# scychon/openmm_drudeNose

Measured on AMD Instinct MI355X. Metric: integrator steps/sec at 1M Drude pairs, higher is better.
Workload: dtype f64; 1 GPU; SWM4-NDP water box, 1000000 molecules = 5000000 particle slots, 1000000 Drude pairs, 1 temperature group (+ molecular-COM and Drude thermostats), TGNH mode, mixed precision, numNHChains=1, hard wall 0.02 nm, harness force call-out inside the timed region (harness_force: lattice); harness_force=lattice, precision=mixed, variant=resident, hipgraph=False, parallelism=particle-sharded x1 (whole molecules), one KE all-reduce per step, slots_per_gpu=5000000

## Files before the change

openmm_drudenose_amd/csrc/tgnh_kernels.hip:

```cpp
#include "tgnh_tile_device.h"

#ifdef TGNH_TRACE
TGNH_TRACE_READERS(tgnh_debug_read_trace, tgnh_debug_clear_trace)
extern "C" int tgnh_debug_read_chain_trace(unsigned long long* out) {
    return (int)hipMemcpyFromSymbol(out, HIP_SYMBOL(tgnh::g_chain_trace), sizeof(unsigned long long) * 8);
}
#endif

namespace tgnh {


size_t tile_lds_bytes(int precision, int ops, bool hardwall, bool use_com) {
    (void)use_com;
    const size_t m4 = (precision == TGNH_PREC_SINGLE) ? 16 : 32;
    const bool hw = hardwall && (ops & (OP_DRIFT | OP_MOVE));
    size_t b = (size_t)(TBLOCK / 64) * (MAX_GROUPS + 2) * 8;
    if ((ops & (OP_SCALE | OP_KE)) || hw) b = m4 * (TILE_SLOTS + TILE_RES);
    if (hw) b += m4 * TILE_SLOTS;
    return b;
}

#ifndef TGNH_MINWAVES
#define TGNH_MINWAVES 1
#endif
// ... 626 lines not shown
            const double dx = ix[pl] - v.x, dy = iy[pl] - v.y, dz = iz[pl] - v.z;
            const double mass1 = mass, mass2 = im[pl];
            const double mu = mass1 * mass2 * rcp_(mass1 + mass2);
            const double d = (dx * dx + dy * dy + dz * dz) * mu;
            ke_drude += d;
            val -= d;
        }
#pragma unroll
        for (int b = 0; b < GB; b++) ke_g[b] += (g == (uint32_t)b) ? val : 0.0;
        __builtin_amdgcn_fence(__ATOMIC_RELEASE, "wavefront");
        __builtin_amdgcn_wave_barrier();
        __builtin_amdgcn_fence(__ATOMIC_ACQUIRE, "wavefront");
    };

    int w = __builtin_amdgcn_readfirstlane((int)blockIdx.x * (TBLOCK / 64) + wv);
    Bounds b0{}, b1{}, b2{};
    WaveIn<PREC> A, B;
    PatternWord pw;
    auto load = [&](const Bounds& b, WaveIn<PREC>& in) {
        const bool patterned = pw.of(a, (uint32_t)b.y >> 8, lane);
        wave_load<PREC, OPS>(a, b.ws, b.n, patterned, pw.word, lane, in);
    };
    if (w < nw) { bounds(w, b0); load(b0, A); }
    if (w + stride < nw) bounds(w + stride, b1);
    while (w < nw) {
        if (w + 2 * stride < nw) bounds(w + 2 * stride, b2);
        if (w + stride < nw) load(b1, B);
        work(A, b0);
        w += stride;
        if (w >= nw) break;
        if (w + 2 * stride < nw) bounds(w + 2 * stride, b0);
        if (w + stride < nw) load(b2, A);
        work(B, b1);
        w += stride;
        b1 = b0; b0 = b2;
    }
#pragma unroll
    for (int b = 0; b < GB; b++) ke_g[b] = wave_sum(ke_g[b]);
    ke_com = wave_sum(ke_com);
    ke_drude = wave_sum(ke_drude);
    if (lane == 0) {
#pragma unroll
        for (int b = 0; b < GB; b++) sred[wv][b] = ke_g[b];
        sred[wv][GB] = ke_com;
        sred[wv][GB + 1] = ke_drude;
    }
    __syncthreads();
    if (tid < GB + 2) {
        double t = 0.0;
#pragma unroll
        for (int k = 0; k < TBLOCK / 64; k++) t += sred[k][tid];
        const int b = tid < GB ? tid : G + (tid - GB);
        if (tid >= GB || tid < G) {
            if (a.tail_sum) {
                unsigned long long* cell = a.rows + row_word((int)blockIdx.x, 2 * b);
                const unsigned long long bits = (unsigned long long)__double_as_longlong(t), tg = (unsigned long long)(gen0 + 1u) << 32;
                __hip_atomic_store(cell, tg | (bits & 0xffffffffull), __ATOMIC_RELAXED, __HIP_MEMORY_SCOPE_SYSTEM);
                __hip_atomic_store(cell + 64, tg | (bits >> 32), __ATOMIC_RELAXED, __HIP_MEMORY_SCOPE_SYSTEM);
            } else a.partials[(size_t)blockIdx.x * (G + 2) + b] = t;
        }
    }
    if (a.tail_sum && blockIdx.x == 0) {
        __shared__ double s_tail[TBLOCK / 64][GB + 2];
        const int NT = G + 2;
        double acc[GB + 2];
#pragma unroll
        for (int b = 0; b < GB + 2; b++) acc[b] = 0.0;
        const bool ok = collect_rows<GB, false, TBLOCK>(a, tid, (int)gridDim.x, NT, (unsigned long long)(gen0 + 1u), acc);
        if (!ok) atomicOr(a.status, 16u);
#pragma unroll
        for (int b = 0; b < GB + 2; b++) {
            if (b < NT) {
                const double t = wave_sum(acc[b]);
                if (lane == 0) s_tail[wv][b] = t;
            }
        }
        const bool all_ok = __syncthreads_and(ok ? 1 : 0) != 0;
        if (tid < NT) {
            double t = 0.0;
#pragma unroll
            for (int k = 0; k < TBLOCK / 64; k++) t += s_tail[k][tid];
            a.ke_red[tid] = all_ok ? t : __longlong_as_double(0x7ff8000000000000ll);
        }
        if (tid == 0) a.sync[1] = gen0 + 1u;
    }
}



enum : int { STEP_DEFER = 0, STEP_PLAIN_BEGIN = 1, STEP_PLAIN_END = 2, STEP_SPLIT_BEGIN = 3, STEP_SPLIT_END = 4, STEP_KINDS = 5 };
constexpr int step_ops1(int kind) {
    return (kind == STEP_DEFER || kind == STEP_PLAIN_END) ? (OP_KICK | OP_KE | OP_NOSTORE) : OP_KE;
}
constexpr int step_ops2(int kind) {
    return kind == STEP_DEFER ? (OP_PREKICK | OP_SCALE | OP_KICK | OP_DRIFT)
         : kind == STEP_PLAIN_BEGIN ? (OP_SCALE | OP_KICK | OP_DRIFT)
         : kind == STEP_PLAIN_END ? (OP_PREKICK | OP_SCALE)
         : kind == STEP_SPLIT_BEGIN ? (OP_SCALE | OP_KICK | OP_POSDELTA)
         : OP_SCALE;
}

template <int PREC, int GB, int KIND>
__global__ __launch_bounds__(TBLOCK, TGNH_MINWAVES) void step_kernel(const TileArgs a) {
    typedef typename Prec<PREC>::mixed mixed;
    constexpr int STEP_OPS1 = step_ops1(KIND), STEP_OPS2 = step_ops2(KIND);
    __shared__ double s_scale[MAX_GROUPS + 2];
    __shared__ double s_part[TBLOCK / 64][CHAIN_INLINE_SUM_NT];
    __shared__ double s_x[64 + XCHG_MAX_WORLD * CHAIN_INLINE_SUM_NT];
    __shared__ int s_go;
    __shared__ unsigned s_gen;
    __shared__ unsigned long long s_seq1;
    extern __shared__ __attribute__((aligned(16))) char smem[];
    const int tid = threadIdx.x, G = a.num_groups, NT = G + 2;
    const int grid = (int)gridDim.x;
    const bool chain_wave = tid < 64;
    const int itg = tid & 63;
    if (a.census) {
        if (tid == 0) {
            __hip_atomic_fetch_add(&a.sync[2], 1u, __ATOMIC_RELAXED, __HIP_MEMORY_SCOPE_AGENT);
            unsigned n = 0;
            while (__hip_atomic_load(&a.sync[2], __ATOMIC_RELAXED, __HIP_MEMORY_SCOPE_AGENT) < gridDim.x && ++n < CENSUS_SPIN_LIMIT)
                __builtin_amdgcn_s_sleep(16);
            if (__hip_atomic_load(&a.sync[2], __ATOMIC_RELAXED, __HIP_MEMORY_SCOPE_AGENT) < gridDim.x) atomicOr(&a.sync[3], 1u);
        }
        return;
    }
    TileEnv<PREC, GB> e;
    e.init(a, smem, s_scale, OpsOf<STEP_OPS2>::POS && a.hardwall != 0);
    auto tile_of = [&](int tt) { return a.reverse ? a.num_tiles - 1 - tt : tt; };

    unsigned gen0 = 0;
    unsigned long long seq0 = 0;
    Chain1Regs creg{};
    if (chain_wave) {
        gen0 = __hip_atomic_load(&a.sync[1], __ATOMIC_RELAXED, __HIP_MEMORY_SCOPE_AGENT);
        seq0 = __hip_atomic_load(a.chain.x.seq, __ATOMIC_RELAXED, __HIP_MEMORY_SCOPE_AGENT);
        if (itg < NT) creg = chain1_load(a.chain, a.st_in, itg);
    }

    TRACE(0);
    TileIn<PREC> cur;
    int tt = blockIdx.x;
    TilePattern tp;
    tile_load<PREC, STEP_OPS1>(a, tile_of(tt), cur, tp);
    for (;;) {
        tile_body<PREC, STEP_OPS1, GB>(a, e, cur, 4);
        if (tt + grid >= a.num_tiles) break;
        tt += grid;
        tile_load<PREC, STEP_OPS1>(a, tile_of(tt), cur, tp);
    }
    const int tt_last = tt;
    TRACE(1);
    MeetShared sh{s_scale, s_part, s_x, &s_go, &s_gen, &s_seq1, nullptr};
    if (!step_meet<PREC, GB>(a, e, gen0, seq0, creg, sh, [&] { tile_load<PREC, STEP_OPS2, STEP_OPS1>(a, tile_of(tt_last), cur, tp); }))
        return;
    e.s_com = (mixed)s_scale[G]; e.s_drude = (mixed)s_scale[G + 1];
    TRACE(9);

    tt = tt_last;
    for (bool held = true;; held = false) {
        tile_body<PREC, STEP_OPS2, GB>(a, e, cur, 0, held);
        if (tt - grid < 0) break;
        tt -= grid;
        tile_load<PREC, STEP_OPS2>(a, tile_of(tt), cur, tp);
    }
    TRACE(15);
}


template <int PREC, int GB, bool MULTI = false>
__global__ __launch_bounds__(WBLOCK) void wstep_kernel(const TileArgs a) {
    typedef typename Prec<PREC>::mixed mixed;
    static_assert(GB > 0, "register bins only");
    __shared__ double s_scale[MAX_GROUPS + 2];
    __shared__ double s_part[WBLOCK / 64][CHAIN_INLINE_SUM_NT];
    __shared__ double s_x[64 + XCHG_MAX_WORLD * CHAIN_INLINE_SUM_NT];
    __shared__ int s_go;
    __shared__ unsigned s_gen;
    __shared__ unsigned long long s_seq1;
    __shared__ mixed s_img[WBLOCK / 64][7][WAVE_SLOTS];
    __shared__ double s_block[256];
    const int tid = threadIdx.x, lane = tid & 63, G = a.num_groups, NT = G + 2;
    const int wv = __builtin_amdgcn_readfirstlane(tid >> 6);
    const bool chain_wave = tid < 64;
    const int itg = tid & 63;
    if (a.census) {
        if (tid == 0) {
            __hip_atomic_fetch_add(&a.sync[2], 1u, __ATOMIC_RELAXED, __HIP_MEMORY_SCOPE_AGENT);
            unsigned n = 0;
            while (__hip_atomic_load(&a.sync[2], __ATOMIC_RELAXED, __HIP_MEMORY_SCOPE_AGENT) < gridDim.x && ++n < CENSUS_SPIN_LIMIT)
                __builtin_amdgcn_s_sleep(16);
            if (__hip_atomic_load(&a.sync[2], __ATOMIC_RELAXED, __HIP_MEMORY_SCOPE_AGENT) < gridDim.x) atomicOr(&a.sync[3], 1u);
        }
        return;
    }
    TileEnv<PREC, GB> e;
    e.tid = tid; e.G = G; e.smem = nullptr; e.wbins0 = nullptr; e.s_scale = s_scale;
    e.clear_ke();
    WaveStep<PREC, GB> ws(a, &e, s_scale, &s_img[wv][0][0], lane);
    typedef WaveBounds Bounds;
    auto bounds = [&](const int ww, Bounds& b) { ws.bounds(ww, b); };
    auto load_vf = [&](const Bounds& b, WStepIn<PREC>& in) { ws.load_vf(b, in); };
    auto load_x = [&](const Bounds& b, WStepIn<PREC>& in) { ws.load_x(b, in); };
    auto prepare = [&](WStepIn<PREC>& t, const Bounds& bd, const bool ke) { ws.template prepare<true>(t, bd, ke); };
    auto finish = [&](WStepIn<PREC>& t, const Bounds& bd) { ws.finish(t, bd); };
    auto wfence = [] { WaveStep<PREC, GB>::wfence(); };

    unsigned gen0 = 0;
    unsigned long long seq0 = 0;
    Chain1Regs creg{};
    if (chain_wave) {
        gen0 = __hip_atomic_load(&a.sync[1], __ATOMIC_RELAXED, __HIP_MEMORY_SCOPE_AGENT);
        seq0 = __hip_atomic_load(a.chain.x.seq, __ATOMIC_RELAXED, __HIP_MEMORY_SCOPE_AGENT);
        if (itg < NT && !(MULTI && a.chain.L.C > 1)) creg = chain1_load(a.chain, a.st_in, itg);
    }
    if (MULTI && a.chain.L.C > 1 && tid < a.chain.L.total) s_block[tid] = a.st_in[tid];

    const int nw = a.num_wtiles, stride = (int)gridDim.x * (WBLOCK / 64);

    TRACE(0);
    const int w0 = __builtin_amdgcn_readfirstlane((int)blockIdx.x * (WBLOCK / 64) + wv);
    const bool have = w0 < nw;
    int w = w0;
    Bounds b0{}, b1{};
    WStepIn<PREC> cur;
    if (have) {
        bounds(w, b0);
        if (w + stride < nw) bounds(w + stride, b1);
        load_vf(b0, cur);
    }
    while (have) {
#ifdef TGNH_TRACE
        if (w == w0) { asm volatile("s_waitcnt vmcnt(0)" ::: "memory"); TRACE(3); }
#endif
        prepare(cur, b0, true);
#ifdef TGNH_TRACE
        if (w == w0) TRACE(4);
#endif
        if (w + stride >= nw) break;
        wfence();
        w += stride;
        b0 = b1;
        if (w + stride < nw) bounds(w + stride, b1);
        load_vf(b0, cur);
    }
    const int w_last = w;
    TRACE(1);
    MeetShared sh{s_scale, s_part, s_x, &s_go, &s_gen, &s_seq1, s_block};
    if (!step_meet<PREC, GB, true, WBLOCK, MULTI>(a, e, gen0, seq0, creg, sh, [&] {
            if (have) {
                load_x(b0, cur);
                if (w_last - stride >= 0) bounds(w_last - stride, b1);
            }
        })) return;

    TRACE(9);
    if (have) {
        w = w_last;
        finish(cur, b0);
        TRACE(5);
        while (w - stride >= 0) {
            w -= stride;
            b0 = b1;
            if (w - stride >= 0) bounds(w - stride, b1);
            load_vf(b0, cur); load_x(b0, cur);
            prepare(cur, b0, false);
            finish(cur, b0);
        }
    }
    TRACE(15);
}

constexpr int CHAIN_LDS_DOUBLES = 2048;

__device__ __forceinline__ void chain_prologue(const ChainArgs& a, double (*sred)[MAX_GROUPS + 2], double* s_chain, double* s_ke) {
    const ChainLayout& L = a.L;
    const int NT = L.NT, tid = threadIdx.x, lane = tid & 63, wv = tid >> 6;
    double* st = a.st;
    if (a.commit) {
        for (int i = tid; i < L.total; i += BLOCK)
            if (i < L.off_ke_red || i >= L.off_ke_red + NT) st[i] = a.stage[i];
        __syncthreads();
    }
    if (a.do_sum) {
        constexpr int PER = GRID_CAP / BLOCK;
        double acc[MAX_GROUPS + 2];
#pragma unroll
        for (int b = 0; b < MAX_GROUPS + 2; b++) acc[b] = 0.0;
        if (NT <= 4) {
            double val[PER][4];
#pragma unroll
            for (int j = 0; j < PER; j++) {
                const int p = tid + j * BLOCK;
#pragma unroll
                for (int b = 0; b < 4; b++) val[j][b] = (p < a.nparts && b < NT) ? a.partials[(size_t)p * NT + b] : 0.0;
            }
#pragma unroll
            for (int j = 0; j < PER; j++)
#pragma unroll
                for (int b = 0; b < 4; b++) acc[b] += val[j][b];
        } else {
#pragma unroll
            for (int b = 0; b < MAX_GROUPS + 2; b++) {
                if (b < NT) {
                    double val[PER];
#pragma unroll
                    for (int j = 0; j < PER; j++) { const int p = tid + j * BLOCK; val[j] = p < a.nparts ? a.partials[(size_t)p * NT + b] : 0.0; }
#pragma unroll
                    for (int j = 0; j < PER; j++) acc[b] += val[j];
                }
            }
        }
        for (int p = tid; p < a.nbig; p += BLOCK) {
#pragma unroll
            for (int b = 0; b < MAX_GROUPS + 2; b++)
                if (b < NT) acc[b] += a.partials[((size_t)GRID_CAP + p) * NT + b];
        }
#pragma unroll
        for (int b = 0; b < MAX_GROUPS + 2; b++) {
            if (b < NT) {
                const double s = wave_sum(acc[b]);
                if (lane == 0) sred[wv][b] = s;
            }
        }
        __syncthreads();
        if (tid < NT) {
            double s = 0.0;
            for (int w = 0; w < BLOCK / 64; w++) s += sred[w][tid];
            st[L.off_ke_red + tid] = s;
            s_ke[tid] = s;
        }
        __syncthreads();
    } else if (tid < NT) {
        s_ke[tid] = st[chain_ke_src(a) + tid];
    }
    if (tid < NT && a.status && !a.ke_carry && s_ke[tid] != s_ke[tid]) atomicOr(a.status, 16u);
    if (a.x_send) xchg_send(a.x, NT, tid, BLOCK, s_chain, tid < NT ? s_ke[tid] : 0.0);
    if (a.x_wait) {
        __syncthreads();
        if (tid < 64) {
            const double tot = xchg_wait_sum(a.x, NT, tid, s_chain);
            if (tid < NT) { s_ke[tid] = tot; st[L.off_ke_red + tid] = tot; }
        }
        __syncthreads();
    }
}

__global__ __launch_bounds__(BLOCK) void rowsum_kernel(const ChainArgs a) {
    __shared__ double sred[BLOCK / 64][MAX_GROUPS + 2];
    __shared__ double s_chain[2 * XCHG_MAX_WORLD * XCHG_NT_PAD > 64 ? 2 * XCHG_MAX_WORLD * XCHG_NT_PAD : 64];
    __shared__ double s_ke[MAX_GROUPS + 2];
    chain_prologue(a, sred, s_chain, s_ke);
}

__global__ __launch_bounds__(BLOCK) void chain_kernel(const ChainArgs a) {
    __shared__ double sred[BLOCK / 64][MAX_GROUPS + 2];
    __shared__ double s_chain[CHAIN_LDS_DOUBLES];
    __shared__ double s_ke[MAX_GROUPS + 2];
    const ChainLayout& L = a.L;
    const int NT = L.NT, tid = threadIdx.x;
    double* st = a.st;
    CHAIN_TRACE(0);
    chain_prologue(a, sred, s_chain, s_ke);
    if (!a.do_chain) return;
    if (!a.do_sum) __syncthreads();
    CHAIN_TRACE(1);
    if (L.mode == TGNH_MODE_TGNH && L.C > 4 && L.C <= 16 && a.lanes) {
        chain_lanes_run(a, st, tid, BLOCK, s_ke);
        if (tid == 0) {
            double s = 0.0;
            for (int i = 0; i < NT; i++) s += s_ke[i];
            st[L.off_kesum] = 0.5 * s;
        }
    } else if (L.mode == TGNH_MODE_TGNH) {
        int itg = -1;
        if (tid < NT - 1) itg = tid;
        else if (tid == 64) itg = NT - 1;
        if (itg >= 0) {
            switch (L.C) {
                case 1: { Chain1Regs r = chain1_load(a, a.st, itg); r.ke = s_ke[itg]; chain1_run(a, r, a.st, true, nullptr, itg); } break;
                case 2: run_tgnh<2>(a, a.st, a.st, true, nullptr, itg, s_chain, s_ke[itg]); break;
                case 3: run_tgnh<3>(a, a.st, a.st, true, nullptr, itg, s_chain, s_ke[itg]); break;
                case 4: run_tgnh<4>(a, a.st, a.st, true, nullptr, itg, s_chain, s_ke[itg]); break;
                default: run_tgnh<0>(a, a.st, a.st, true, nullptr, itg, s_chain, s_ke[itg]); break;
            }
        }
        if (tid == 0) {
            double s = 0.0;
            for (int i = 0; i < NT; i++) s += s_ke[i];
            st[L.off_kesum] = 0.5 * s;
        }
    } else if (L.C == 1) {
        if (tid < 3) {
            Chain1Regs r = chain1_load(a, a.st, tid); r.ke = s_ke[tid];
            if (L.c1_quirk) chain1q_run(a, r, a.st, true, nullptr, tid);
            else chain1_run(a, r, a.st, true, nullptr, tid);
        }
        if (tid == 64) st[L.off_kesum] = 0.5 * (s_ke[0] + s_ke[2]);
    } else if (tid == 0) {
        switch (L.C) {
            case 1: run_dualnh<1>(a, a.st, a.st, true, nullptr, s_chain, s_ke[0], s_ke[1], s_ke[2]); break;
            case 2: run_dualnh<2>(a, a.st, a.st, true, nullptr, s_chain, s_ke[0], s_ke[1], s_ke[2]); break;
            case 3: run_dualnh<3>(a, a.st, a.st, true, nullptr, s_chain, s_ke[0], s_ke[1], s_ke[2]); break;
            case 4: run_dualnh<4>(a, a.st, a.st, true, nullptr, s_chain, s_ke[0], s_ke[1], s_ke[2]); break;
            default: run_dualnh<0>(a, a.st, a.st, true, nullptr, s_chain, s_ke[0], s_ke[1], s_ke[2]); break;
        }
    }
    CHAIN_TRACE(2);
}
template <int CC>
__global__ __launch_bounds__(BLOCK) void chain_long_kernel(const ChainArgs a) {
    __shared__ double sred[BLOCK / 64][MAX_GROUPS + 2];
    __shared__ double s_chain[2 * XCHG_MAX_WORLD * XCHG_NT_PAD > 64 ? 2 * XCHG_MAX_WORLD * XCHG_NT_PAD : 64];
// ... 565 lines not shown
```

openmm_drudenose_amd/csrc/tgnh_tile_device.h:

```cpp
#ifndef TGNH_TILE_DEVICE_H_
#define TGNH_TILE_DEVICE_H_
#include "tgnh_internal.h"

namespace tgnh {
__device__ __forceinline__ double wave_sum(double v);
#ifdef TGNH_TRACE
static __device__ unsigned long long g_trace[GRID_CAP * 16];
#define TRACE(slot) do { if (threadIdx.x == 0 && (slot) < 16) g_trace[blockIdx.x * 16 + (slot)] = wall_clock64(); } while (0)
#define TRACE_WAIT() __builtin_amdgcn_s_waitcnt(0)
#define TGNH_TRACE_READERS(read_name, clear_name)                                                            \
    extern "C" int read_name(unsigned long long* out) {                                                      \
        return (int)hipMemcpyFromSymbol(out, HIP_SYMBOL(tgnh::g_trace), sizeof(unsigned long long) * tgnh::GRID_CAP * 16); \
    }                                                                                                        \
    extern "C" int clear_name() {                                                                            \
        void* p = nullptr;                                                                                   \
        if (hipGetSymbolAddress(&p, HIP_SYMBOL(tgnh::g_trace)) != hipSuccess) return 1;                      \
        return (int)hipMemset(p, 0, sizeof(unsigned long long) * tgnh::GRID_CAP * 16);                       \
    }
static __device__ __attribute__((unused)) unsigned long long g_chain_trace[8];
#define CHAIN_TRACE(slot) do { if (threadIdx.x == 0) { g_chain_trace[2 * (slot)] = wall_clock64(); g_chain_trace[2 * (slot) + 1] = clock64(); } } while (0)
#else
#define TRACE(slot) do {} while (0)
#define TRACE_WAIT() do {} while (0)
#define CHAIN_TRACE(slot) do {} while (0)
// ... 69 lines not shown
        else img[i] = u;
    }
    __device__ __forceinline__ static mixed4 ld_img(const mixed4* img, int i) {
        const mixed* imgc = reinterpret_cast<const mixed*>(img);
        if (SOA) return mk4(imgc[i], imgc[TILE_SLOTS + i], imgc[2 * TILE_SLOTS + i], imgc[3 * TILE_SLOTS + i]);
        return img[i];
    }
    __device__ __forceinline__ void init(const TileArgs& a, char* smem_, double* s_scale_, bool hardwall_lds) {
        smem = smem_; s_scale = s_scale_;
        sv = reinterpret_cast<mixed4*>(smem); scom = sv + TILE_SLOTS; sx = scom + TILE_RES;
        tid = threadIdx.x; G = a.num_groups; use_com = a.use_com != 0;
        dt = (mixed)a.dt;
        fscale = (mixed)(0.5 * a.dt / 4294967296.0);
        s_com = 1; s_drude = 1;
        wbins0 = reinterpret_cast<double*>(sx + (hardwall_lds ? TILE_SLOTS : 0));
        clear_ke();
    }
    __device__ __forceinline__ void clear_ke() {
#pragma unroll
        for (int b = 0; b < GBR; b++) ke_g[b] = 0.0;
        ke_com = 0.0; ke_drude = 0.0;
        if (GB == 0) { double* w = wbins0 + (tid >> 6) * G; for (int g = tid & 63; g < G; g += 64) w[g] = 0.0; }
    }
};

__device__ __forceinline__ size_t row_word(const int r, const int j) {
    return ((size_t)(r >> 6) * (2 * CHAIN_INLINE_SUM_NT) + j) * 64 + (r & 63);
}

template <int PREC, int GB, bool TAGGED, int NTH = TBLOCK>
__device__ __forceinline__ void ke_reduce(const TileArgs& a, TileEnv<PREC, GB>& e, const unsigned tag = 0u, double* scratch = nullptr) {
    typedef TileEnv<PREC, GB> E;
    const int tid = e.tid, G = e.G;
    double (&ke_g)[E::GBR] = e.ke_g;
    double ke_com = e.ke_com, ke_drude = e.ke_drude;
    auto put = [&](const int b, double v) {
        if (TAGGED) {
            unsigned long long* cell = a.rows + row_word((int)blockIdx.x, 2 * b);
            const unsigned long long bits = (unsigned long long)__double_as_longlong(v), t = (unsigned long long)tag << 32;
            __hip_atomic_store(cell, t | (bits & 0xffffffffull), __ATOMIC_RELAXED, __HIP_MEMORY_SCOPE_SYSTEM);
            __hip_atomic_store(cell + 64, t | (bits >> 32), __ATOMIC_RELAXED, __HIP_MEMORY_SCOPE_SYSTEM);
        } else a.partials[(size_t)blockIdx.x * (G + 2) + b] = v;
    };
    double* sred = scratch ? scratch : reinterpret_cast<double*>(e.smem);
    const int lane = tid & 63, wv = tid >> 6;
#pragma unroll
    for (int b = 0; b < GB; b++) ke_g[b] = wave_sum(ke_g[b]);
    if (GB == 0) __syncthreads();
    ke_com = wave_sum(ke_com);
    ke_drude = wave_sum(ke_drude);
    if (lane == 0) {
#pragma unroll
        for (int b = 0; b < GB; b++) sred[wv * (GB + 2) + b] = ke_g[b];
        sred[wv * (GB + 2) + GB] = ke_com;
        sred[wv * (GB + 2) + GB + 1] = ke_drude;
    }
    __syncthreads();
    if (tid < GB + 2) {
        double s = 0.0;
#pragma unroll
        for (int w = 0; w < NTH / 64; w++) s += sred[w * (GB + 2) + tid];
        if (tid < GB) { if (tid < G) put(tid, s); }
        else put(G + (tid - GB), s);
    }
    if (GB == 0) {
        const double* w0 = e.wbins0;
        for (int g = tid; g < G; g += NTH) {
            double s = 0.0;
#pragma unroll
            for (int w = 0; w < NTH / 64; w++) s += w0[w * G + g];
            put(g, s);
        }
    }
}

__device__ __forceinline__ double force_as(const long long f, double) {
    return fma((double)(int)(f >> 32), 4294967296.0, (double)(unsigned)f);
}
__device__ __forceinline__ float force_as(const long long f, float) { return (float)f; }

struct PatternWord {
    uint32_t pat = 0u, word = 0u;
    __device__ __forceinline__ bool of(const TileArgs& a, const uint32_t p, const int lane) {
        if ((p & 255u) == 0u) return false;
        if (p != pat) {
            const int period = (int)(p & 255u);
            const int q = (int)(((float)lane + 0.5f) * __builtin_amdgcn_rcpf((float)period));
            word = a.wpattern[(p >> 8) * PATTERN_WORDS + (uint32_t)(lane - q * period)];
            pat = p;
        }
        return true;
    }
};

template <int GB, bool LEAN, int NTH>
__device__ __forceinline__ bool collect_rows(const TileArgs& a, const int tid, const int grid, const int NT, const unsigned long long want,
                                             double (&acc)[GB + 2]) {
    constexpr int NTM = GB + 2;
    bool ok = true;
        constexpr int RB = (GB == 1 && !LEAN) ? 3 : 1, CH = 3;
#pragma unroll 1
        for (int r0 = tid; r0 < grid && ok; r0 += RB * NTH) {
#pragma unroll 1
            for (int b0 = 0; b0 < NT && ok; b0 += CH) {
                unsigned long long w[RB][2 * CH];
                bool have[RB];
#pragma unroll
                for (int k = 0; k < RB; k++) have[k] = r0 + k * NTH >= grid;
                unsigned n = 0;
                for (;;) {
#pragma unroll
                    for (int k = 0; k < RB; k++) {
                        if (!have[k]) {
                            const unsigned long long* cell = a.rows + row_word(r0 + k * NTH, 2 * b0);
#pragma unroll
                            for (int b = 0; b < 2 * CH; b++) if (b0 + b / 2 < NT) w[k][b] = xchg_ld(cell + b * 64);
                        }
                    }
                    bool all = true;
#pragma unroll
                    for (int k = 0; k < RB; k++) {
                        if (!have[k]) {
                            bool row = true;
#pragma unroll
                            for (int b = 0; b < 2 * CH; b++) if (b0 + b / 2 < NT) row = row && (w[k][b] >> 32) == want;
                            have[k] = row;
                        }
                        all = all && have[k];
                    }
                    if (all) break;
                    if (++n > XCHG_SPIN_LIMIT) { ok = false; break; }
                }
#pragma unroll
                for (int k = 0; k < RB; k++)
#pragma unroll
                    for (int b = 0; b < CH; b++)
                        if (b0 + b < NT && r0 + k * NTH < grid) {
                            const double v = __longlong_as_double((long long)((w[k][2 * b + 1] << 32) | (w[k][2 * b] & 0xffffffffull)));
#pragma unroll
                            for (int t = 0; t < NTM; t++) acc[t] += (t == b0 + b) ? v : 0.0;
                        }
            }
        }
    return ok;
}

struct MeetShared {
    double* s_scale;
    double (*s_part)[CHAIN_INLINE_SUM_NT];
    double* s_x;
    int* s_go_p; unsigned* s_gen_p; unsigned long long* s_seq1_p;
    const double* s_block;
};
template <int PREC, int GB, bool LEAN = false, int NTH = TBLOCK, bool MULTI = false, typename Prefetch>
__device__ __forceinline__ bool step_meet(const TileArgs& a, TileEnv<PREC, GB>& e, const unsigned gen0, const unsigned long long seq0,
                                          Chain1Regs& creg, const MeetShared& sh, Prefetch&& prefetch) {
    double* const s_scale = sh.s_scale; double (*const s_part)[CHAIN_INLINE_SUM_NT] = sh.s_part; double* const s_x = sh.s_x;
    int& s_go = *sh.s_go_p; unsigned& s_gen = *sh.s_gen_p; unsigned long long& s_seq1 = *sh.s_seq1_p;
    const int tid = threadIdx.x, G = a.num_groups, NT = G + 2, grid = (int)gridDim.x;
    const bool chain_wave = tid < 64, leader = blockIdx.x == 0;
    const int itg = tid & 63;
    const ChainLayout& L = a.chain.L;
    if (chain_wave) asm volatile("" :: "v"(creg.eta), "v"(creg.etaDot0), "v"(creg.etaDot1), "v"(creg.etaDotDot), "v"(creg.etaMass), "v"(creg.nkbt) : "memory");
    ke_reduce<PREC, GB, true, NTH>(a, e, gen0 + 1u, s_x);
    TRACE(2);
    prefetch();
    constexpr bool EARLY_PRE = PREC != TGNH_PREC_SINGLE && !LEAN;
    Chain1Pre cpre{};
    if (EARLY_PRE && chain_wave && !L.c1_quirk && !(MULTI && L.C > 1)) cpre = chain1_prepare(a.chain, creg, itg);

    if (tid == 0) { s_gen = gen0; s_seq1 = seq0 + 1ull; }
    __syncthreads();
    const unsigned long long want = (unsigned long long)(s_gen + 1u);
    if (leader) {
        unsigned long long* const my_peer = xchg_peer_of(a.chain.x, tid);
        constexpr int NTM = GB + 2;
        double acc[NTM];
#pragma unroll
        for (int b = 0; b < NTM; b++) acc[b] = 0.0;
        bool ok = true;
        TRACE(6);
        ok = collect_rows<GB, LEAN, NTH>(a, tid, grid, NT, want, acc);
        TRACE(10);
        if (!ok) {
            atomicOr(a.status, 8u);
            __hip_atomic_store(a.chain.x.dead, 1u, __ATOMIC_RELAXED, __HIP_MEMORY_SCOPE_AGENT);
        }
        const double* big = a.partials + (size_t)GRID_CAP * NT;
        for (int r = tid; r < a.chain.nbig; r += NTH)
#pragma unroll
            for (int b = 0; b < NTM; b++) if (b < NT) acc[b] += big[(size_t)r * NT + b];
#pragma unroll
        for (int b = 0; b < NTM; b++) {
            if (b < NT) {
                const double t = wave_sum(acc[b]);
                if ((tid & 63) == 0) s_part[tid >> 6][b] = t;
            }
        }
        const bool all_ok = __syncthreads_and(ok ? 1 : 0) != 0;
        TRACE(7);
        const XchgArgs& x = a.chain.x;
        const unsigned long long seq = s_seq1, stag = (seq & 0xffffffffull) << 32;
        if (tid == 0) { a.sync[1] = s_gen + 1u; *x.seq = seq; }
        const int tpp = NTH / x.world;
        if (all_ok && tid < tpp * x.world) {
            unsigned long long* const base = my_peer + xchg_cell(x, (unsigned)(seq & 1ull), x.rank, 0, 0);
            for (int q = tid / x.world; q < NT * XCHG_REPLICAS; q += tpp) {
                const int copy = q / NT, i = q - copy * NT;
                double v = 0.0;
#pragma unroll
                for (int w = 0; w < NTH / 64; w++) v += s_part[w][i];
                const unsigned long long bits = (unsigned long long)__double_as_longlong(v);
                unsigned long long* cell = base + (size_t)copy * XCHG_REPLICA_U64 + (size_t)i * XCHG_CELL_U64;
                __hip_atomic_store(cell, stag | (bits & 0xffffffffull), __ATOMIC_RELAXED, __HIP_MEMORY_SCOPE_SYSTEM);
                __hip_atomic_store(cell + 1, stag | (bits >> 32), __ATOMIC_RELAXED, __HIP_MEMORY_SCOPE_SYSTEM);
            }
        }
        TRACE(13);
    }
    if (chain_wave) {
        bool dead = false;
        const double mine = xchg_wait_sum<true>(a.chain.x, NT, itg, s_x + 64, seq0 + 1ull, &dead);
        TRACE(8);
        if (itg == 0) s_go = dead ? 0 : 1;
        if (!dead) {
            const bool write = leader;
            creg.ke = mine;
            if (write && itg < NT) a.st_out[L.off_ke_red + itg] = mine;
            if (write) {
                const double kesum = wave_sum(itg < NT ? mine : 0.0);
                if (itg == 63) a.st_out[L.off_kesum] = 0.5 * kesum;
            }
            if (MULTI && L.C > 1) chainN_run<false>(a.chain, sh.s_block, a.st_out, write, s_scale, itg, mine);
            else if (itg < NT) {
                if (L.c1_quirk) chain1q_run(a.chain, creg, a.st_out, write, s_scale, itg);
                else chain1_finish(a.chain, creg, EARLY_PRE ? cpre : chain1_prepare(a.chain, creg, itg), a.st_out, write, s_scale, itg);
            }
        }
    }
    __syncthreads();
    return s_go != 0;
}

template <int PREC> struct WStepIn {
    typename Prec<PREC>::mixed4 v;
    uint32_t meta;
    long long fx, fy, fz;
    typename Prec<PREC>::real4 p;
    float4 c;
    typename Prec<PREC>::mixed mass, cx, cy, cz;
};

struct WaveBounds { int ws, y, n; };

template <int PREC, int GB> struct WaveStep {
    typedef typename Prec<PREC>::real real;
    typedef typename Prec<PREC>::mixed mixed;
    typedef typename Prec<PREC>::real4 real4;
    typedef typename Prec<PREC>::mixed4 mixed4;
    const TileArgs& a;
    TileEnv<PREC, GB>* e;
    const double* s_scale;
    mixed *ix, *iy, *iz, *im, *jx, *jy, *jz;
    mixed4* __restrict__ velm; real4* __restrict__ posq; float4* __restrict__ pcorr;
    int lane, G, nw;
    bool use_com, hardwall;
    mixed dt, fscale;
    PatternWord pw;
    __device__ __forceinline__ WaveStep(const TileArgs& a_, TileEnv<PREC, GB>* e_, const double* s_scale_, mixed* img, const int lane_)
        : a(a_), e(e_), s_scale(s_scale_), ix(img), iy(img + WAVE_SLOTS), iz(img + 2 * WAVE_SLOTS), im(img + 3 * WAVE_SLOTS),
          jx(img + 4 * WAVE_SLOTS), jy(img + 5 * WAVE_SLOTS), jz(img + 6 * WAVE_SLOTS),
          velm(reinterpret_cast<mixed4*>(a_.velm)), posq(reinterpret_cast<real4*>(a_.posq)), pcorr(reinterpret_cast<float4*>(a_.posq_corr)),
          lane(lane_), G(a_.num_groups), nw(a_.num_wtiles), use_com(a_.use_com != 0), hardwall(a_.hardwall != 0),
          dt((mixed)a_.dt), fscale((mixed)(0.5 * a_.dt / 4294967296.0)) {}
    __device__ __forceinline__ static void wfence() {
        __builtin_amdgcn_fence(__ATOMIC_RELEASE, "wavefront");
        __builtin_amdgcn_wave_barrier();
        __builtin_amdgcn_fence(__ATOMIC_ACQUIRE, "wavefront");
    }
    __device__ __forceinline__ void bounds(const int ww, WaveBounds& b) const {
        const int2* t = a.wave_tile + (a.reverse ? nw - 1 - ww : ww);
        b.ws = t[0].x; b.y = t[0].y; b.n = t[1].x - b.ws;
    }
    __device__ __forceinline__ void load_vf(const WaveBounds& b, WStepIn<PREC>& in) {
        const int idx = b.ws + lane;
        const bool patterned = pw.of(a, (uint32_t)b.y >> 8, lane);
        mixed4 v = mk4((mixed)0, (mixed)0, (mixed)0, (mixed)0);
        uint32_t meta = 64u << 10;
        long long fx = 0, fy = 0, fz = 0;
        if (lane < b.n) {
            v = reinterpret_cast<const mixed4*>(a.velm)[idx];
            if (!patterned) meta = a.wmeta[idx];
            fx = a.force[idx]; fy = a.force[idx + a.padded]; fz = a.force[idx + 2 * a.padded];
        }
        if (patterned && lane < b.n) meta = pw.word;
        in.v = v; in.meta = meta; in.fx = fx; in.fy = fy; in.fz = fz;
    }
    __device__ __forceinline__ void load_x(const WaveBounds& b, WStepIn<PREC>& in) const {
        const int idx = b.ws + lane;
        if (lane < b.n) {
            in.p = reinterpret_cast<const real4*>(a.posq)[idx];
            if (PREC == TGNH_PREC_MIXED) in.c = reinterpret_cast<const float4*>(a.posq_corr)[idx];
        }
    }
    template <bool KICK = true>
    __device__ __forceinline__ void prepare(WStepIn<PREC>& t, const WaveBounds& bd, const bool ke) {
        mixed4& v = t.v;
        const uint32_t m = t.meta;
        t.mass = v.w != 0 ? rcp_(v.w) : (mixed)0;
        if (KICK) {
            const mixed c = fscale * v.w;
            v.x += c * force_as(t.fx, (mixed)0);
            v.y += c * force_as(t.fy, (mixed)0);
            v.z += c * force_as(t.fz, (mixed)0);
        }
        ix[lane] = v.x; iy[lane] = v.y; iz[lane] = v.z; im[lane] = t.mass;
        wfence();
        mixed cx = 0, cy = 0, cz = 0;
        if (use_com) {
            const int j = (int)((m >> 17) & 63u), n1 = (int)((m >> 23) & 63u);
            const int first = lane - j;
            mixed px = 0, py = 0, pz = 0, pm = 0;
            for (int k = 0; k < (bd.y & 255); k++) {
                if (k <= n1) {
                    const mixed um = im[first + k];
                    px += ix[first + k] * um; py += iy[first + k] * um; pz += iz[first + k] * um; pm += um;
                }
            }
            const mixed wq = rcp_(pm);
            cx = px * wq; cy = py * wq; cz = pz * wq;
            if (ke && j == 0 && lane < bd.n)
                e->ke_com += ((double)cx * cx + (double)cy * cy + (double)cz * cz) * (double)pm;
        }
        t.cx = cx; t.cy = cy; t.cz = cz;
        if (ke) {
            const uint32_t role = m & 3u, g = (m >> 2) & 255u;
            const double rx = v.x - cx, ry = v.y - cy, rz = v.z - cz;
            double val = v.w != 0 ? (rx * rx + ry * ry + rz * rz) * (double)t.mass : 0.0;
            if (role == ROLE_DRUDE) {
                const int pl = lane + (int)((m >> 10) & 127u) - 64;
                const double dx = ix[pl] - v.x, dy = iy[pl] - v.y, dz = iz[pl] - v.z;
                const double mass1 = t.mass, mass2 = im[pl];
                const double mu = mass1 * mass2 * rcp_(mass1 + mass2);
                const double d = (dx * dx + dy * dy + dz * dz) * mu;
                e->ke_drude += d;
                val -= d;
            }
#pragma unroll
            for (int b = 0; b < GB; b++) e->ke_g[b] += (g == (uint32_t)b) ? val : 0.0;
        }
    }
    __device__ __forceinline__ void finish(WStepIn<PREC>& t, const WaveBounds& bd) {
        mixed4 v = t.v;
        const uint32_t m = t.meta;
        const uint32_t role = m & 3u, g = (m >> 2) & 255u;
        const int pl = lane + (int)((m >> 10) & 127u) - 64;
        const mixed mass = t.mass, cx = t.cx, cy = t.cy, cz = t.cz;
        const mixed s_com = (mixed)s_scale[G], s_drude = (mixed)s_scale[G + 1], s_g = (mixed)s_scale[g];
        mixed px = t.p.x, py = t.p.y, pz = t.p.z;
        const real pq = t.p.w;
        if (PREC == TGNH_PREC_MIXED) { px += (mixed)t.c.x; py += (mixed)t.c.y; pz += (mixed)t.c.z; }
        if (role == ROLE_NORMAL) {
            if (v.w != 0) {
                const mixed rx = v.x - cx, ry = v.y - cy, rz = v.z - cz;
                v.x = s_g * rx + s_com * (v.x - rx);
                v.y = s_g * ry + s_com * (v.y - ry);
                v.z = s_g * rz + s_com * (v.z - rz);
            }
        } else {
            const mixed ux = ix[pl], uy = iy[pl], uz = iz[pl], um = im[pl];
            const mixed rsx = v.x - cx, rsy = v.y - cy, rsz = v.z - cz;
            const mixed rpx = ux - cx, rpy = uy - cy, rpz = uz - cz;
            const mixed invTot = rcp_(mass + um);
            const mixed msf = invTot * mass, mpf = invTot * um;
            const mixed sdp = s_drude * mpf;
            v.x = s_g * (rsx * msf + rpx * mpf) + sdp * (rsx - rpx) + s_com * (v.x - rsx);
            v.y = s_g * (rsy * msf + rpy * mpf) + sdp * (rsy - rpy) + s_com * (v.y - rsy);
            v.z = s_g * (rsz * msf + rpz * mpf) + sdp * (rsz - rpz) + s_com * (v.z - rsz);
        }
        if (v.w != 0) {
            const mixed c = fscale * v.w;
            v.x += c * force_as(t.fx, (mixed)0);
            v.y += c * force_as(t.fy, (mixed)0);
            v.z += c * force_as(t.fz, (mixed)0);
            px += dt * v.x; py += dt * v.y; pz += dt * v.z;
        }
        if (hardwall) {
            wfence();
            ix[lane] = v.x; iy[lane] = v.y; iz[lane] = v.z;
            jx[lane] = px; jy[lane] = py; jz[lane] = pz;
            wfence();
            if (role != ROLE_NORMAL) {
                const mixed maxd = (mixed)a.max_dist, hws = (mixed)a.hw_scale;
                const mixed sxd = px - jx[pl], syd = py - jy[pl], szd = pz - jz[pl];
                const mixed d2 = sxd * sxd + syd * syd + szd * szd;
                if (d2 > maxd * maxd) {
                    const mixed4 uv = mk4(ix[pl], iy[pl], iz[pl], im[pl]);
                    const bool is_d = role == ROLE_DRUDE;
                    const mixed4 vel1 = is_d ? v : uv, vel2 = is_d ? uv : v;
                    const mixed dx = is_d ? sxd : -sxd, dy = is_d ? syd : -syd, dz = is_d ? szd : -szd;
                    const mixed r = sqrt_(d2);
                    const mixed rInv = rcp_(r);
                    if (rInv * maxd < (mixed)0.5) atomicOr(a.status, 1u);
                    const mixed bx = dx * rInv, by = dy * rInv, bz = dz * rInv;
                    const mixed mass1 = is_d ? mass : uv.w, mass2 = is_d ? uv.w : mass;
                    const mixed deltaR = r - maxd;
                    mixed deltaT = dt;
                    mixed dotvr1 = vel1.x * bx + vel1.y * by + vel1.z * bz;
                    const mixed vp1x = vel1.x - bx * dotvr1, vp1y = vel1.y - by * dotvr1, vp1z = vel1.z - bz * dotvr1;
                    const mixed invTot = rcp_(mass1 + mass2);
                    mixed dotvr2 = vel2.x * bx + vel2.y * by + vel2.z * bz;
                    const mixed vp2x = vel2.x - bx * dotvr2, vp2y = vel2.y - by * dotvr2, vp2z = vel2.z - bz * dotvr2;
                    const mixed vbCMass = (mass1 * dotvr1 + mass2 * dotvr2) * invTot;
                    dotvr1 -= vbCMass;
                    dotvr2 -= vbCMass;
                    if (dotvr1 != dotvr2) deltaT = deltaR / abs_(dotvr1 - dotvr2);
                    if (deltaT > dt) deltaT = dt;
                    const mixed vBond = hws / sqrt_(mass1);
                    dotvr1 = -dotvr1 * vBond * mass2 * invTot / abs_(dotvr1);
                    dotvr2 = -dotvr2 * vBond * mass1 * invTot / abs_(dotvr2);
                    const mixed dr1 = -deltaR * mass2 * invTot + deltaT * dotvr1;
                    const mixed dr2 = deltaR * mass1 * invTot + deltaT * dotvr2;
                    dotvr1 += vbCMass;
                    dotvr2 += vbCMass;
                    if (is_d) {
                        px += bx * dr1; py += by * dr1; pz += bz * dr1;
                        v.x = vp1x + bx * dotvr1; v.y = vp1y + by * dotvr1; v.z = vp1z + bz * dotvr1;
                    } else {
                        px += bx * dr2; py += by * dr2; pz += bz * dr2;
                        v.x = vp2x + bx * dotvr2; v.y = vp2y + by * dotvr2; v.z = vp2z + bz * dotvr2;
                    }
                }
            }
        }
        wfence();
        if (lane < bd.n) {
            const int idx = bd.ws + lane;
            velm[idx] = v;
            if (PREC == TGNH_PREC_MIXED) {
                const float hx = (float)px, hy = (float)py, hz = (float)pz;
                posq[idx] = mk4((real)hx, (real)hy, (real)hz, pq);
                pcorr[idx] = make_float4((float)(px - hx), (float)(py - hy), (float)(pz - hz), 0.0f);
            } else {
                posq[idx] = mk4((real)px, (real)py, (real)pz, pq);
            }
        }
    }
};

}
#endif
```

Measured before the change: 4364 steps/s.

## Stage next wave's inputs into LDS during the step barrier wait

While non-leader, non-chain waves wait at the global step meet, they issue asynchronous global-to-LDS loads (global_load_lds) for the next reverse-pass wave chunk: velocities, forces, positions, corrections and meta. After the meet, non-zero waves consume that chunk from LDS instead of reloading it from global memory. The point is to hide second-pass load latency behind the barrier spin. It adds a per-wave LDS staging buffer, which may reduce occupancy, and depends on the async LDS writes being visible before they are read.

```diff
diff --git a/openmm_drudenose_amd/csrc/tgnh_kernels.hip b/openmm_drudenose_amd/csrc/tgnh_kernels.hip
--- a/openmm_drudenose_amd/csrc/tgnh_kernels.hip
+++ b/openmm_drudenose_amd/csrc/tgnh_kernels.hip
@@ -802,7 +802,7 @@
     const int tt_last = tt;
     TRACE(1);
     MeetShared sh{s_scale, s_part, s_x, &s_go, &s_gen, &s_seq1, nullptr};
-    if (!step_meet<PREC, GB>(a, e, gen0, seq0, creg, sh, [&] { tile_load<PREC, STEP_OPS2, STEP_OPS1>(a, tile_of(tt_last), cur, tp); }))
+    if (!step_meet<PREC, GB>(a, e, gen0, seq0, creg, sh, [&] { tile_load<PREC, STEP_OPS2, STEP_OPS1>(a, tile_of(tt_last), cur, tp); }, [] {}))
         return;
     e.s_com = (mixed)s_scale[G]; e.s_drude = (mixed)s_scale[G + 1];
     TRACE(9);
@@ -830,6 +830,8 @@
     __shared__ unsigned long long s_seq1;
     __shared__ mixed s_img[WBLOCK / 64][7][WAVE_SLOTS];
     __shared__ double s_block[256];
+    constexpr bool STAGE = TGNH_WSTEP_STAGE != 0;
+    __shared__ __attribute__((aligned(16))) char s_stage[WBLOCK / 64][STAGE ? WStage<PREC>::BYTES : 16];
     const int tid = threadIdx.x, lane = tid & 63, G = a.num_groups, NT = G + 2;
     const int wv = __builtin_amdgcn_readfirstlane(tid >> 6);
     const bool chain_wave = tid < 64;
@@ -897,11 +899,14 @@
     const int w_last = w;
     TRACE(1);
     MeetShared sh{s_scale, s_part, s_x, &s_go, &s_gen, &s_seq1, s_block};
+    char* const slot = &s_stage[wv][0];
     if (!step_meet<PREC, GB, true, WBLOCK, MULTI>(a, e, gen0, seq0, creg, sh, [&] {
             if (have) {
                 load_x(b0, cur);
                 if (w_last - stride >= 0) bounds(w_last - stride, b1);
             }
+        }, [&] {
+            if (STAGE && have && w_last - stride >= 0) ws.stage(b1, slot);
         })) return;
 
     TRACE(9);
@@ -909,6 +914,14 @@
         w = w_last;
         finish(cur, b0);
         TRACE(5);
+        if (STAGE && wv != 0 && w - stride >= 0) {
+            w -= stride;
+            b0 = b1;
+            if (w - stride >= 0) bounds(w - stride, b1);
+            ws.load_staged(b0, cur, slot);
+            prepare(cur, b0, false);
+            finish(cur, b0);
+        }
         while (w - stride >= 0) {
             w -= stride;
             b0 = b1;
diff --git a/openmm_drudenose_amd/csrc/tgnh_tile_device.h b/openmm_drudenose_amd/csrc/tgnh_tile_device.h
--- a/openmm_drudenose_amd/csrc/tgnh_tile_device.h
+++ b/openmm_drudenose_amd/csrc/tgnh_tile_device.h
@@ -245,9 +245,9 @@
     int* s_go_p; unsigned* s_gen_p; unsigned long long* s_seq1_p;
     const double* s_block;
 };
-template <int PREC, int GB, bool LEAN = false, int NTH = TBLOCK, bool MULTI = false, typename Prefetch>
+template <int PREC, int GB, bool LEAN = false, int NTH = TBLOCK, bool MULTI = false, typename Prefetch, typename Stage>
 __device__ __forceinline__ bool step_meet(const TileArgs& a, TileEnv<PREC, GB>& e, const unsigned gen0, const unsigned long long seq0,
-                                          Chain1Regs& creg, const MeetShared& sh, Prefetch&& prefetch) {
+                                          Chain1Regs& creg, const MeetShared& sh, Prefetch&& prefetch, Stage&& stage) {
     double* const s_scale = sh.s_scale; double (*const s_part)[CHAIN_INLINE_SUM_NT] = sh.s_part; double* const s_x = sh.s_x;
     int& s_go = *sh.s_go_p; unsigned& s_gen = *sh.s_gen_p; unsigned long long& s_seq1 = *sh.s_seq1_p;
     const int tid = threadIdx.x, G = a.num_groups, NT = G + 2, grid = (int)gridDim.x;
@@ -265,6 +265,7 @@
     if (tid == 0) { s_gen = gen0; s_seq1 = seq0 + 1ull; }
     __syncthreads();
     const unsigned long long want = (unsigned long long)(s_gen + 1u);
+    if (!leader && !chain_wave) stage();
     if (leader) {
         unsigned long long* const my_peer = xchg_peer_of(a.chain.x, tid);
         constexpr int NTM = GB + 2;
@@ -310,6 +311,7 @@
             }
         }
         TRACE(13);
+        if (!chain_wave) stage();
     }
     if (chain_wave) {
         bool dead = false;
@@ -345,6 +347,36 @@
 };
 
 struct WaveBounds { int ws, y, n; };
+
+#ifndef TGNH_WSTEP_STAGE
+#define TGNH_WSTEP_STAGE 1
+#endif
+
+template <int SIZE, int CAP>
+__device__ __forceinline__ void lds_copy(const void* src, char* dst, const int bytes, const int lane) {
+    static_assert(SIZE == 4 || SIZE == 16, "4 or 16 bytes per lane");
+    typedef __attribute__((address_space(1))) void gvoid;
+    typedef __attribute__((address_space(3))) void lvoid;
+#pragma unroll
+    for (int k = 0; k * 64 * SIZE < CAP; k++) {
+        const int off = k * 64 * SIZE + lane * SIZE;
+        gvoid* const g = (gvoid*)(reinterpret_cast<const char*>(src) + off);
+        lvoid* const l = (lvoid*)(dst + k * 64 * SIZE);
+        if (off < bytes) {
+            if constexpr (SIZE == 16) __builtin_amdgcn_global_load_lds(g, l, 16, 0, 0);
+            else __builtin_amdgcn_global_load_lds(g, l, 4, 0, 0);
+        }
+    }
+}
+
+template <int PREC> struct WStage {
+    static constexpr int V = 0;
+    static constexpr int F = V + WAVE_SLOTS * (int)sizeof(typename Prec<PREC>::mixed4);
+    static constexpr int P = F + 3 * WAVE_SLOTS * (int)sizeof(long long);
+    static constexpr int C = P + WAVE_SLOTS * (int)sizeof(typename Prec<PREC>::real4);
+    static constexpr int M = C + (PREC == TGNH_PREC_MIXED ? WAVE_SLOTS * (int)sizeof(float4) : 0);
+    static constexpr int BYTES = M + WAVE_SLOTS * (int)sizeof(uint32_t);
+};
 
 template <int PREC, int GB> struct WaveStep {
     typedef typename Prec<PREC>::real real;
@@ -395,6 +427,34 @@
             in.p = reinterpret_cast<const real4*>(a.posq)[idx];
             if (PREC == TGNH_PREC_MIXED) in.c = reinterpret_cast<const float4*>(a.posq_corr)[idx];
         }
+    }
+    __device__ __forceinline__ void stage(const WaveBounds& b, char* slot) {
+        typedef WStage<PREC> S;
+        pw.of(a, (uint32_t)b.y >> 8, lane);
+        const int ws = b.ws, n = b.n;
+        lds_copy<16, WAVE_SLOTS * (int)sizeof(mixed4)>(velm + ws, slot + S::V, n * (int)sizeof(mixed4), lane);
+#pragma unroll
+        for (int d = 0; d < 3; d++)
+            lds_copy<4, WAVE_SLOTS * 8>(a.force + ws + d * a.padded, slot + S::F + d * WAVE_SLOTS * 8, n * 8, lane);
+        lds_copy<16, WAVE_SLOTS * (int)sizeof(real4)>(posq + ws, slot + S::P, n * (int)sizeof(real4), lane);
+        if (PREC == TGNH_PREC_MIXED) lds_copy<16, WAVE_SLOTS * 16>(pcorr + ws, slot + S::C, n * 16, lane);
+        if ((((uint32_t)b.y >> 8) & 255u) == 0u) lds_copy<4, WAVE_SLOTS * 4>(a.wmeta + ws, slot + S::M, n * 4, lane);
+    }
+    __device__ __forceinline__ void load_staged(const WaveBounds& b, WStepIn<PREC>& in, const char* slot) const {
+        typedef WStage<PREC> S;
+        const bool patterned = (((uint32_t)b.y >> 8) & 255u) != 0u;
+        mixed4 v = mk4((mixed)0, (mixed)0, (mixed)0, (mixed)0);
+        uint32_t meta = 64u << 10;
+        long long fx = 0, fy = 0, fz = 0;
+        if (lane < b.n) {
+            v = reinterpret_cast<const mixed4*>(slot + S::V)[lane];
+            meta = patterned ? pw.word : reinterpret_cast<const uint32_t*>(slot + S::M)[lane];
+            const long long* f = reinterpret_cast<const long long*>(slot + S::F);
+            fx = f[lane]; fy = f[WAVE_SLOTS + lane]; fz = f[2 * WAVE_SLOTS + lane];
+            in.p = reinterpret_cast<const real4*>(slot + S::P)[lane];
+            if (PREC == TGNH_PREC_MIXED) in.c = reinterpret_cast<const float4*>(slot + S::C)[lane];
+        }
+        in.v = v; in.meta = meta; in.fx = fx; in.fy = fy; in.fz = fz;
     }
     template <bool KICK = true>
     __device__ __forceinline__ void prepare(WStepIn<PREC>& t, const WaveBounds& bd, const bool ke) {
```

Measured after the change: 4383 steps/s (median of 6 runs). Within noise of the previous version (+0.4%).
